# jim-berend/semanticlens

Measured on AMD Instinct MI355X. Metric: images/sec concept-db build, higher is better.
Workload: dtype f32 (encoder GEMMs split-bf16x3, fp32 accumulate)

## Files before the change

include/semanticlens_amd.h:

```cpp
#ifndef SEMANTICLENS_AMD_H
#define SEMANTICLENS_AMD_H

#include <stddef.h>
#include <stdint.h>

#ifdef __cplusplus
extern "C" {
#endif

#define SL_ABI_VERSION 1

#define SL_E_INVALID (-1)
#define SL_E_HIP (-2)
#define SL_E_UNSUPPORTED (-3)

#define SL_F32 0
#define SL_F16 1
#define SL_BF16 2

#define SL_CONV_MAX 0
#define SL_CONV_MEAN 1
#define SL_CONV_SUM 2

#define SL_TOK_MEAN 0
// ... 170 lines not shown
int sl_preprocess_plan_rois(const int32_t* h_hw, const int64_t* h_pixel_offsets, int64_t N, const int64_t* h_index,
                            const int32_t* h_box, int64_t P, int S, int resize_mode, int interp, int64_t* h_plan,
                            int64_t* h_info);

#define SL_RENDER_CROP 0
#define SL_RENDER_OPAQUE 1
#define SL_RENDER_LIGHTEN 2
size_t sl_render_ws_bytes(int64_t B, int64_t H, int64_t W);
int sl_render_heatmaps(const float* d_rel, int64_t B, int64_t Cin, int64_t H, int64_t W, const float* d_img, int kernel_size,
                       float vis_th, float crop_th, double alpha, int style, int rf, float* d_heat, int32_t* d_box,
                       int32_t* d_flags, uint8_t* d_rgb, void* d_ws, size_t ws_bytes, void* stream);
int sl_condition_init(const float* d_act, int64_t B, int64_t C, int64_t S, int64_t sb, int64_t sc, int64_t ss,
                      const int64_t* d_channels, int rf, float* d_out, int64_t ob, int64_t oc, int64_t os, void* stream);

int sl_activation_heat_boxes(const float* d_act, int64_t B, int64_t C, int64_t S, int64_t sb, int64_t sc, int64_t ss,
                             int64_t prefix, int64_t gh, int64_t gw, const int64_t* d_rows, const int64_t* d_channels,
                             int64_t P, int64_t H, int64_t W, int kernel_size, float crop_th, float* d_heat, int32_t* d_box,
                             void* d_ws, size_t ws_bytes, void* stream);
int sl_heat_boxes(const float* d_heat, int64_t P, int64_t H, int64_t W, int kernel_size, float crop_th, int32_t* d_box,
                  void* d_ws, size_t ws_bytes, void* stream);

int sl_batchnorm_infer(const float* d_x, int64_t B, int64_t C, int64_t HW, const float* d_mean, const float* d_var,
                       const float* d_scale, const float* d_bias, double eps, int relu, float* d_y, void* stream);
int sl_batchnorm_infer_add_relu(const float* d_x, const float* d_residual, int64_t B, int64_t C, int64_t HW,
                                const float* d_mean, const float* d_var, const float* d_scale, const float* d_bias,
                                double eps, float* d_y, void* stream);
int sl_batchnorm_infer_add_bn_relu(const float* d_xa, const float* d_mean_a, const float* d_var_a, const float* d_scale_a,
                                   const float* d_bias_a, double eps_a, const float* d_xb, const float* d_mean_b,
                                   const float* d_var_b, const float* d_scale_b, const float* d_bias_b, double eps_b, int64_t B,
                                   int64_t C, int64_t HW, float* d_y, void* stream);
int sl_batchnorm_infer_relu_maxpool(const float* d_x, int64_t B, int64_t C, int64_t H, int64_t W, const float* d_mean,
                                    const float* d_var, const float* d_scale, const float* d_bias, double eps, int kh, int kw,
                                    int sh, int sw, int ph, int pw, float* d_y, void* stream);

int sl_topk_init(float* d_vals, int64_t* d_ids, int64_t R, int64_t k, void* stream);
int sl_topk_merge(float* d_vals, int64_t* d_ids, int64_t R, int64_t k, const float* d_cand, int64_t ld, int64_t B,
                  int64_t id_base, void* d_ws, size_t ws_bytes, void* stream);
size_t sl_topk_merge_ws_bytes(int64_t R, int64_t k, int64_t B);
int sl_topk_merge_states(float* d_vals, int64_t* d_ids, int64_t R, int64_t k, const float* d_other_vals,
                         const int64_t* d_other_ids, int64_t M, void* stream);

int sl_mutualmax_merge(uint64_t* d_row_state, uint64_t* d_col_state, int64_t R, int64_t B, const float* d_cand, int64_t ld,
                       int64_t row_id_base, int64_t col_id_base, void* stream);
int sl_mutualmax_finish(const uint64_t* d_state, int64_t n, float* d_vals, int64_t* d_ids, void* stream);

int sl_segmax_merge(uint64_t* d_state, int64_t state_ld, int64_t G, int64_t R, int64_t B, const float* d_cand, int64_t ld,
                    const int32_t* d_row_seg, int64_t row_id_base, void* stream);

int sl_unionfind_init(int32_t* d_parent, int32_t* d_degree, int32_t* d_status, int64_t n, void* stream);
int sl_threshold_union_merge(int32_t* d_parent, int32_t* d_degree, int32_t* d_status, int64_t n, const float* d_cand, int64_t ld,
                             int64_t R, int64_t B, int64_t row_id_base, int64_t col_id_base, float threshold, void* stream);
int sl_unionfind_flatten(int32_t* d_parent, int64_t n, int32_t* d_status, void* stream);
int sl_group_min_merge(uint32_t* d_state, const int32_t* d_labels, int64_t n, const float* d_cand, int64_t ld, int64_t R, int64_t B,
                       int64_t row_id_base, int64_t col_id_base, void* stream);
int sl_group_min_finish(const uint32_t* d_state, const int32_t* d_labels, int64_t n, float* d_cohesion, void* stream);

int sl_cosine_nt(const float* d_x, int64_t M, const float* d_y, int64_t N, int64_t K, float* d_out, void* d_ws,
                 size_t ws_bytes, void* stream);
size_t sl_cosine_nt_ws_bytes(int64_t M, int64_t N, int64_t K);

#define SL_PROF_REDUCE 0
#define SL_PROF_MERGE 1
#define SL_PROF_GEMM 2
#define SL_PROF_GATHER 3
#define SL_PROF_SCORES 4
#define SL_PROF_BATCHNORM 5
// ... 11 lines not shown
```

semanticlens_amd/_native.py:

```python
from __future__ import annotations

import ctypes
import math
import operator
import os
from pathlib import Path

import torch

_PKG = Path(__file__).resolve().parent
LIB_PATH = _PKG / "lib" / "libsemanticlens_hip.so"

SL_F32, SL_F16, SL_BF16 = 0, 1, 2
SL_CONV_MAX, SL_CONV_MEAN, SL_CONV_SUM = 0, 1, 2
SL_TOK_MEAN, SL_TOK_ABSMEAN, SL_TOK_MAX, SL_TOK_ABSMAX, SL_TOK_TOKEN = 0, 1, 2, 3, 4
SL_TIES_TOTAL, SL_TIES_ATEN = 0, 1
SL_MAX_SLOTS = 16
SL_PROF_REDUCE, SL_PROF_MERGE, SL_PROF_GEMM, SL_PROF_GATHER, SL_PROF_SCORES, SL_PROF_BATCHNORM, SL_PROF_TOPK = 0, 1, 2, 3, 4, 5, 6
SL_ACT_NONE, SL_ACT_GELU, SL_ACT_QUICKGELU, SL_ACT_GELU_TANH = 0, 1, 2, 3
TIE_MODES = {"total": SL_TIES_TOTAL, "aten": SL_TIES_ATEN}
SL_PP_PLAN_STRIDE = 16
PP_RESIZE_MODES = {"shortest": 0, "squash": 1}
PP_INTERP = {"bicubic": 0, "bilinear": 1}
SL_RENDER_CROP, SL_RENDER_OPAQUE, SL_RENDER_LIGHTEN = 0, 1, 2
# ... 60 lines not shown
    "sl_polykmeans_labels": (_int, [_vp, _i64, _i64, _i64, _int, _vp, _int, _vp, _int, _vp, _vp, _vp, _vp, _sz, _vp]),
    "sl_facet_stats": (_int, [_vp, _i64, _i64, _i64, _vp, _int, _vp, _vp, _vp, _vp]),
    "sl_silhouette_ws_bytes": (_sz, [_i64, _i64, _i64]),
    "sl_silhouette": (_int, [_vp, _i64, _i64, _i64, _vp, _int, _int, _int, _vp, _vp, _vp, _sz, _vp]),
    "sl_linear": (_int, [_vp, _i64, _i64, _vp, _i64, _vp, _int, _vp, _vp, _i64, _i64, _i64, _i64, _vp, _vp]),
    "sl_layernorm": (_int, [_vp, _i64, _i64, _i64, _vp, _vp, ctypes.c_float, _vp, _vp, _i64, _vp]),
    "sl_attention": (_int, [_vp, _i64, _i64, _i64, _i64, _int, _vp, _vp, _vp]),
    "sl_attention_bf16x3": (_int, [_vp, _i64, _i64, _i64, _i64, _int, _vp, _vp, _vp]),
    "sl_patchify": (_int, [_vp, _i64, _i64, _i64, _i64, _i64, _vp, _vp, _vp]),
    "sl_attention_pool": (_int, [_vp, _vp, _i64, _i64, _i64, _i64, _i64, _i64, _vp, _vp]),
    "sl_attention_pool_q": (_int, [_vp, _i64, _vp, _i64, _i64, _i64, _i64, _i64, _i64, _vp, _vp]),
    "sl_tokens_from_map": (_int, [_vp, _i64, _i64, _i64, _vp, _vp, _vp]),
    "sl_split_elems": (_sz, [_i64, _i64]),
    "sl_split_bf16": (_int, [_vp, _vp, _i64, _i64, _vp, _vp]),
    "sl_linear_bf16x3": (_int, [_vp, _i64, _i64, _vp, _i64, _vp, _int, _vp, _vp, _vp, _i64, _i64, _i64, _i64, _vp, _vp]),
    "sl_broadcast_row": (_int, [_vp, _vp, _i64, _i64, _i64, _vp, _vp]),
    "sl_embed_tokens": (_int, [_vp, _i64, _vp, _i64, _i64, _i64, _vp, _vp, _vp]),
    "sl_preprocess_plan": (_int, [_vp, _vp, _i64, _int, _int, _int, _vp, _vp]),
    "sl_preprocess": (_int, [_vp, _vp, _i64, _int, _int, _i64, _i64, _vp, _vp, _vp, _vp, _vp, _sz, _vp]),
    "sl_render_ws_bytes": (_sz, [_i64, _i64, _i64]),
    "sl_render_heatmaps": (_int, [_vp, _i64, _i64, _i64, _i64, _vp, _int, ctypes.c_float, ctypes.c_float, ctypes.c_double, _int, _int,
                                  _vp, _vp, _vp, _vp, _vp, _sz, _vp]),
    "sl_condition_init": (_int, [_vp, _i64, _i64, _i64, _i64, _i64, _i64, _vp, _int, _vp, _i64, _i64, _i64, _vp]),
    "sl_preprocess_plan_rois": (_int, [_vp, _vp, _i64, _vp, _vp, _i64, _int, _int, _int, _vp, _vp]),
    "sl_activation_heat_boxes": (_int, [_vp, _i64, _i64, _i64, _i64, _i64, _i64, _i64, _i64, _i64, _vp, _vp, _i64, _i64, _i64, _int,
                                        ctypes.c_float, _vp, _vp, _vp, _sz, _vp]),
    "sl_heat_boxes": (_int, [_vp, _i64, _i64, _i64, _int, ctypes.c_float, _vp, _vp, _sz, _vp]),
    "sl_batchnorm_infer": (_int, [_vp, _i64, _i64, _i64, _vp, _vp, _vp, _vp, ctypes.c_double, _int, _vp, _vp]),
    "sl_batchnorm_infer_add_relu": (_int, [_vp, _vp, _i64, _i64, _i64, _vp, _vp, _vp, _vp, ctypes.c_double, _vp, _vp]),
    "sl_batchnorm_infer_add_bn_relu": (_int, [_vp, _vp, _vp, _vp, _vp, ctypes.c_double, _vp, _vp, _vp, _vp, _vp, ctypes.c_double, _i64, _i64,
                                              _i64, _vp, _vp]),
    "sl_batchnorm_infer_relu_maxpool": (_int, [_vp, _i64, _i64, _i64, _i64, _vp, _vp, _vp, _vp, ctypes.c_double, _int, _int, _int,
                                               _int, _int, _int, _vp, _vp]),
    "sl_topk_init": (_int, [_vp, _vp, _i64, _i64, _vp]),
    "sl_topk_merge": (_int, [_vp, _vp, _i64, _i64, _vp, _i64, _i64, _i64, _vp, _sz, _vp]),
    "sl_topk_merge_ws_bytes": (_sz, [_i64, _i64, _i64]),
    "sl_topk_merge_states": (_int, [_vp, _vp, _i64, _i64, _vp, _vp, _i64, _vp]),
    "sl_mutualmax_merge": (_int, [_vp, _vp, _i64, _i64, _vp, _i64, _i64, _i64, _vp]),
    "sl_mutualmax_finish": (_int, [_vp, _i64, _vp, _vp, _vp]),
    "sl_segmax_merge": (_int, [_vp, _i64, _i64, _i64, _i64, _vp, _i64, _vp, _i64, _vp]),
    "sl_unionfind_init": (_int, [_vp, _vp, _vp, _i64, _vp]),
    "sl_threshold_union_merge": (_int, [_vp, _vp, _vp, _i64, _vp, _i64, _i64, _i64, _i64, _i64, ctypes.c_float, _vp]),
    "sl_unionfind_flatten": (_int, [_vp, _i64, _vp, _vp]),
    "sl_group_min_merge": (_int, [_vp, _vp, _i64, _vp, _i64, _i64, _i64, _i64, _i64, _vp]),
    "sl_group_min_finish": (_int, [_vp, _vp, _i64, _vp, _vp]),
    "sl_cosine_nt": (_int, [_vp, _i64, _vp, _i64, _i64, _vp, _vp, _sz, _vp]),
    "sl_cosine_nt_ws_bytes": (_sz, [_i64, _i64, _i64]),
    "sl_prof_enable": (_int, [_int]),
    "sl_prof_reset": (_int, []),
    "sl_prof_read": (_int, [_int, ctypes.POINTER(ctypes.c_double), ctypes.POINTER(_i64), ctypes.POINTER(ctypes.c_double)]),
}

_lib = None


class NativeLibraryError(RuntimeError):
    """The HIP library is missing or a native call failed."""


def lib():
    global _lib
    if _lib is None:
        path = Path(os.environ.get("SEMANTICLENS_AMD_LIB", LIB_PATH))
        if not path.exists():
            raise NativeLibraryError(
                f"{path} not found. semanticlens_amd has no CPU fallback: build the HIP library first "
# ... 950 lines not shown
        if residual is None:
            rc = lib().sl_batchnorm_infer(_ptr(x), B, C, H * W, _ptr(mean), _ptr(var), _ptr(weight), _ptr(bias), float(eps),
                                          1 if relu else 0, _ptr(out), _stream(x))
        else:
            rc = lib().sl_batchnorm_infer_add_relu(_ptr(x), _ptr(residual), B, C, H * W, _ptr(mean), _ptr(var), _ptr(weight),
                                                   _ptr(bias), float(eps), _ptr(out), _stream(x))
    _check(rc, "sl_batchnorm_infer")
    return out


BN_DUAL_MAX_CHANNELS = 2048


def batchnorm_infer_add_bn_relu(xa: torch.Tensor, bn_a, xb: torch.Tensor, bn_b) -> torch.Tensor:
    if xa.shape != xb.shape or xa.dim() != 4 or xa.device != xb.device:
        raise ValueError(f"batchnorm_infer_add_bn_relu: two 4-D tensors of one shape and device expected, got {tuple(xa.shape)} and "
                         f"{tuple(xb.shape)}")
    B, C, H, W = xa.shape
    for t in (xa, xb):
        if t.dtype is not torch.float32 or not t.is_contiguous() or t.data_ptr() % 16:
            raise ValueError("batchnorm_infer_add_bn_relu: inputs must be contiguous NCHW fp32, 16-byte aligned")
    for p in (*bn_a[:4], *bn_b[:4]):
        if p.dtype is not torch.float32 or p.device != xa.device or not p.is_contiguous() or p.numel() != C:
            raise ValueError(f"batchnorm_infer_add_bn_relu: per-channel tensors must be contiguous fp32 of {C} elements on {xa.device}")
    out = torch.empty_like(xa)
    with _on(xa.device):
        rc = lib().sl_batchnorm_infer_add_bn_relu(_ptr(xa), *(_ptr(p) for p in bn_a[:4]), float(bn_a[4]), _ptr(xb),
                                                  *(_ptr(p) for p in bn_b[:4]), float(bn_b[4]), B, C, H * W, _ptr(out), _stream(xa))
    _check(rc, "sl_batchnorm_infer_add_bn_relu")
    return out


BN_POOL_MAX_WIDTH = 4096
BN_POOL_STAGE_BYTES = 64 * 1024


def bn_pool_supported(kernel_size, stride, padding) -> bool:
    return all(k in (2, 3) and s in (1, 2) and 0 <= p <= k // 2 for k, s, p in zip(kernel_size, stride, padding))


def batchnorm_infer_relu_maxpool(x: torch.Tensor, mean: torch.Tensor, var: torch.Tensor, weight: torch.Tensor, bias: torch.Tensor,
                                 eps: float, kernel_size, stride, padding) -> torch.Tensor:
    B, C, H, W = x.shape
    (kh, kw), (sh, sw), (ph, pw) = kernel_size, stride, padding
    oh, ow = ((n + 2 * p - k) // s + 1 if s > 0 else 0 for n, k, s, p in ((H, kh, sh, ph), (W, kw, sw, pw)))
    out = torch.empty((B, C, max(oh, 0), max(ow, 0)), dtype=x.dtype, device=x.device)
    with _on(x.device):
        rc = lib().sl_batchnorm_infer_relu_maxpool(_ptr(x), B, C, H, W, _ptr(mean), _ptr(var), _ptr(weight), _ptr(bias),
                                                   float(eps), kh, kw, sh, sw, ph, pw, _ptr(out), _stream(x))
    _check(rc, "sl_batchnorm_infer_relu_maxpool")
    return out


def prof_enable(on: bool = True):
    _check(lib().sl_prof_enable(1 if on else 0), "sl_prof_enable")


def prof_reset():
    _check(lib().sl_prof_reset(), "sl_prof_reset")


def prof_read(family: int):
    ms, n, w = ctypes.c_double(), _i64(), ctypes.c_double()
    _check(lib().sl_prof_read(family, ctypes.byref(ms), ctypes.byref(n), ctypes.byref(w)), "sl_prof_read")
    return ms.value, n.value, w.value


POLY2_MAX_N = 128


POLYK_MAX_N = 1024
# ... 522 lines not shown
```

semanticlens_amd/component_visualization/_bn_fuse.py:

```python
from __future__ import annotations

import inspect
import operator
import os
import warnings
import weakref

import torch
import torch.nn as nn
import torch.nn.functional as F

from .. import _native as N

_BN_FORWARD = nn.modules.batchnorm._BatchNorm.forward
_PLANS: "weakref.WeakKeyDictionary[nn.Module, _Plan]" = weakref.WeakKeyDictionary()
_ADDS = (operator.add, operator.iadd, torch.add)
_RELUS = (F.relu, torch.relu, torch.relu_)
_POOL_ARGS = ("kernel_size", "stride", "padding", "dilation", "ceil_mode", "return_indices")


def enabled() -> bool:
    return os.environ.get("SEMANTICLENS_AMD_FUSE_BN", "1") != "0"


# ... 63 lines not shown
            if p is None or p.dtype is not torch.float32 or p.device != x.device or not p.is_contiguous() or p.numel() != x.shape[1]:
                return False
        return True

    def run(self, x, relu: bool, other=None, bn_first: bool = True):
        bn = self.bn
        out = N.batchnorm_infer(x, bn.running_mean, bn.running_var, bn.weight, bn.bias, bn.eps, relu=relu, residual=other)
        key = (relu, other is not None, (x.shape[2] * x.shape[3]) % 4 == 0)
        if key in self.verified:
            return out
        ref = F.batch_norm(x, bn.running_mean, bn.running_var, bn.weight, bn.bias, False, 0.0, bn.eps)
        if other is not None:
            ref = ref + other if bn_first else other + ref
        if relu:
            ref = torch.relu_(ref)
        if torch.equal(out.view(torch.int32), ref.view(torch.int32)):
            self.verified.add(key)
            return out
        self.dropped = True
        warnings.warn(
            f"the fused BatchNorm kernel did not reproduce PyTorch's result bit for bit on a {tuple(x.shape)} input "
            f"(relu={relu}, residual={other is not None}); this BatchNorm2d runs unfused from now on.", RuntimeWarning, stacklevel=3)
        return ref

    def pool_eligible(self, x, params) -> bool:
        (kh, kw), _, (ph, pw) = params
        return (not self.no_pool and x.shape[3] <= N.BN_POOL_MAX_WIDTH and x.shape[2] + 2 * ph >= kh
                and x.shape[3] + 2 * pw >= kw)

    def run_pool(self, x, params):
        bn = self.bn
        k, s, p = params
        out = N.batchnorm_infer_relu_maxpool(x, bn.running_mean, bn.running_var, bn.weight, bn.bias, bn.eps, k, s, p)
        banded = x.shape[2] > N.BN_POOL_STAGE_BYTES // (4 * x.shape[3])
        key = ("pool", params, x.shape[3] % 4 == 0 and out.shape[3] % 4 == 0, banded)
        if key in self.verified:
            return out
        ref = F.batch_norm(x, bn.running_mean, bn.running_var, bn.weight, bn.bias, False, 0.0, bn.eps)
        ref = F.max_pool2d(torch.relu_(ref), k, s, p)
        if out.shape == ref.shape and torch.equal(out.view(torch.int32), ref.view(torch.int32)):
            self.verified.add(key)
            return out
        self.no_pool = True
        warnings.warn(
            f"the fused BatchNorm + ReLU + max-pool kernel did not reproduce PyTorch's result bit for bit on a {tuple(x.shape)} "
            f"input (kernel_size={k}, stride={s}, padding={p}); this max-pool runs unfused from now on.", RuntimeWarning,
            stacklevel=3)
        return ref


def _bn_args(bn: nn.BatchNorm2d):
    return bn.running_mean, bn.running_var, bn.weight, bn.bias, bn.eps


def _bn_forward(site: _Site):
    def forward(x):
        if site.eligible(x):
            return site.run(x, relu=False)
        return _BN_FORWARD(site.bn, x)

    return forward


class _Fused(nn.Module):

    def __init__(self, site: _Site, relu, add=None, bn_first: bool = True):
        super().__init__()
        self.__dict__.update(site=site, relu=relu, add=add, bn_first=bn_first)
# ... 249 lines not shown
```

semanticlens_amd/csrc/batchnorm.hip:

```cpp
#include "common.hpp"

namespace sl {
namespace {

typedef float f4 __attribute__((ext_vector_type(4)));

enum { EPI_PLAIN = 0, EPI_RELU = 1, EPI_ADD_RELU = 2, EPI_ADD_BN_RELU = 3 };
enum { POL_PLAIN = 0, POL_NT_STORE = 1, POL_NT_BOTH = 2 };

constexpr int kBlock = 256;
constexpr int kUnroll = 4;
constexpr int64_t kMaxC = 4096;
constexpr int64_t kMaxCDual = 2048;
constexpr int64_t kLdsPerCu = 160 * 1024;
constexpr size_t kDualResidentFrom = 32 * 1024;
constexpr int64_t kMaxTotal = (int64_t)1 << 31;

__device__ inline float bn_inv_std(float var, double eps) { return __builtin_amdgcn_rsqf(fabsf(var + (float)eps)); }

__device__ inline float bn_value(float x, const f4 k) {
  const float xhat = (x - k.x) * k.y;
  return __fmaf_rn(k.z, xhat, k.w);
}

__device__ inline float relu_clamp(float v) { return v != v ? v : fmaxf(v, 0.f); }

__device__ inline float add_as_aten(float a, float b) {
  float r;
  asm("v_add_f32_e32 %0, %1, %2" : "=v"(r) : "v"(b), "v"(a));
  return r;
}

struct BnParams {
// ... 147 lines not shown
  ProfScope prof(SL_PROF_BATCHNORM, st, (double)total * 4 * passes);
  const int pol = bn_policy(total * 4);
  const size_t lds = (size_t)C * sizeof(f4) * (dual ? 2 : 1);
  const int64_t per_block = (int64_t)kBlock * kUnroll * 4;
  int64_t blocks = (total + per_block - 1) / per_block;
  int64_t per_cu = 8;
  if (dual && lds > kDualResidentFrom) per_cu = kLdsPerCu / (int64_t)lds;
  const int64_t cap = (int64_t)num_cus() * per_cu;
  if (blocks > cap) blocks = cap;
  const dim3 grid((unsigned)blocks);
#define SL_BN_EPI(E_)                                                                                                \
  if (HW % 4 == 0)                                                                                                   \
    launch_policy<E_, true>(prof, pol, grid, lds, st, x, res, y, a, b, (uint32_t)C, (uint32_t)HW, (uint32_t)total);  \
  else                                                                                                               \
    launch_policy<E_, false>(prof, pol, grid, lds, st, x, res, y, a, b, (uint32_t)C, (uint32_t)HW, (uint32_t)total)
  switch (epi) {
    case EPI_PLAIN: SL_BN_EPI(EPI_PLAIN); break;
    case EPI_RELU: SL_BN_EPI(EPI_RELU); break;
    case EPI_ADD_RELU: SL_BN_EPI(EPI_ADD_RELU); break;
    default: SL_BN_EPI(EPI_ADD_BN_RELU); break;
  }
#undef SL_BN_EPI
  SL_CHECK_HIP(hipGetLastError());
  if (dual) {
    ProfScope second(SL_PROF_BATCHNORM, st, 0.0);
    if (second.start) {
      SL_CHECK_HIP(hipEventRecord(second.start, st));
      SL_CHECK_HIP(hipEventRecord(second.stop, st));
    }
  }
  return 0;
}

constexpr int64_t kPoolLds = 64 * 1024;
constexpr int64_t kPoolMaxW = 4096;

struct PoolGeom {
  uint32_t C, H, W, OH, OW, kh, kw, sh, sw, ph, pw;
  uint32_t rows, bands;
  uint32_t nwork;
};

struct PoolBand {
  uint32_t plane, o0, o1, r0, r1;
  f4 k;
};

__device__ inline PoolBand pool_band(const PoolGeom& g, uint32_t work, const float* mean, const float* var, const float* scale,
                                     const float* bias, double eps) {
  PoolBand b;
  b.plane = work / g.bands;
  const uint32_t band = work - b.plane * g.bands, c = b.plane % g.C;
  b.k = f4{mean[c], bn_inv_std(var[c], eps), scale[c], bias[c]};
  b.o0 = band * g.rows;
  b.o1 = b.o0 + g.rows < g.OH ? b.o0 + g.rows : g.OH;
  const int top = (int)(b.o0 * g.sh) - (int)g.ph;
  b.r0 = top > 0 ? (uint32_t)top : 0u;
  const uint32_t bottom = (b.o1 - 1) * g.sh + g.kh - g.ph;
  b.r1 = bottom < g.H ? bottom : g.H;
  return b;
}

__device__ inline float pool_take(float m, float v) { return v > m || v != v ? v : m; }

template <int KW, int SW, int PW, int POL>
__global__ __launch_bounds__(kBlock) void bn_relu_maxpool_kernel(const float* __restrict__ x, float* __restrict__ y,
                                                                 const float* __restrict__ mean, const float* __restrict__ var,
                                                                 const float* __restrict__ scale, const float* __restrict__ bias,
                                                                 double eps, const PoolGeom g) {
  extern __shared__ f4 staged[];
  for (uint32_t work = blockIdx.x; work < g.nwork; work += gridDim.x) {
    const PoolBand b = pool_band(g, work, mean, var, scale, bias, eps);
    const uint32_t w4 = g.W / 4, n4 = (b.r1 - b.r0) * w4;
    const f4* src = reinterpret_cast<const f4*>(x + (size_t)b.plane * g.H * g.W) + (size_t)b.r0 * w4;
    for (uint32_t base = 0; base < n4; base += kBlock * kUnroll) {
      f4 v[kUnroll];
#pragma unroll
      for (int u = 0; u < kUnroll; ++u) {
        const uint32_t i = base + u * kBlock + threadIdx.x;
        if (i < n4) v[u] = ld4<POL>(src + i);
      }
#pragma unroll
      for (int u = 0; u < kUnroll; ++u) {
        const uint32_t i = base + u * kBlock + threadIdx.x;
        if (i < n4) {
          f4 o;
#pragma unroll
          for (int j = 0; j < 4; ++j) o[j] = relu_clamp(bn_value(v[u][j], b.k));
          staged[i] = o;
        }
      }
    }
    __syncthreads();

    constexpr int OFF = PW ? 3 : 0, SPAN = 3 * SW + KW, PIECES = (OFF + SPAN + 3) / 4;
    constexpr float NEG_INF = -__builtin_huge_valf();
    const uint32_t ow4 = g.OW / 4, npieces = (b.o1 - b.o0) * ow4;
    f4* dst = reinterpret_cast<f4*>(y + (size_t)b.plane * g.OH * g.OW);
    for (uint32_t p = threadIdx.x; p < npieces; p += kBlock) {
      const uint32_t orow = p / ow4, q = p - orow * ow4, oh = b.o0 + orow;
      const int col0 = (int)(q * 4 * SW) - (PW ? 4 : 0);
      f4 m = {NEG_INF, NEG_INF, NEG_INF, NEG_INF};
#pragma unroll
      for (int i = 0; i < 3; ++i) {
        const int ih = (int)(oh * g.sh) - (int)g.ph + i;
        if (i < (int)g.kh && ih >= 0 && ih < (int)g.H) {
          const f4* row = staged + (size_t)((uint32_t)ih - b.r0) * w4;
          float t[PIECES * 4];
#pragma unroll
          for (int s = 0; s < PIECES; ++s) {
            const int col = col0 + 4 * s;
            const f4 piece = col >= 0 && col < (int)g.W ? row[col >> 2] : f4{NEG_INF, NEG_INF, NEG_INF, NEG_INF};
#pragma unroll
            for (int j = 0; j < 4; ++j) t[4 * s + j] = piece[j];
          }
#pragma unroll
          for (int o = 0; o < 4; ++o) {
#pragma unroll
            for (int j = 0; j < KW; ++j) m[o] = pool_take(m[o], t[OFF + o * SW + j]);
          }
        }
      }
      st4<POL>(dst + (size_t)oh * ow4 + q, m);
    }
    __syncthreads();
  }
}

template <int POL>
__global__ __launch_bounds__(kBlock) void bn_relu_maxpool_scalar_kernel(const float* __restrict__ x, float* __restrict__ y,
                                                                        const float* __restrict__ mean,
                                                                        const float* __restrict__ var,
                                                                        const float* __restrict__ scale,
                                                                        const float* __restrict__ bias, double eps,
                                                                        const PoolGeom g) {
  extern __shared__ f4 staged[];
  float* rows = reinterpret_cast<float*>(staged);
  for (uint32_t work = blockIdx.x; work < g.nwork; work += gridDim.x) {
    const PoolBand b = pool_band(g, work, mean, var, scale, bias, eps);
    const uint32_t n = (b.r1 - b.r0) * g.W;
    const float* src = x + (size_t)b.plane * g.H * g.W + (size_t)b.r0 * g.W;
#pragma unroll 4
    for (uint32_t i = threadIdx.x; i < n; i += kBlock) rows[i] = relu_clamp(bn_value(ld1<POL>(src + i), b.k));
    __syncthreads();

    const uint32_t nout = (b.o1 - b.o0) * g.OW;
    float* dst = y + (size_t)b.plane * g.OH * g.OW;
    for (uint32_t p = threadIdx.x; p < nout; p += kBlock) {
      const uint32_t orow = p / g.OW, ow = p - orow * g.OW, oh = b.o0 + orow;
      float m = -__builtin_huge_valf();
      for (uint32_t i = 0; i < g.kh; ++i) {
        const int ih = (int)(oh * g.sh) - (int)g.ph + (int)i;
        if (ih < 0 || ih >= (int)g.H) continue;
        for (uint32_t j = 0; j < g.kw; ++j) {
          const int iw = (int)(ow * g.sw) - (int)g.pw + (int)j;
          if (iw < 0 || iw >= (int)g.W) continue;
          m = pool_take(m, rows[((uint32_t)ih - b.r0) * g.W + (uint32_t)iw]);
        }
      }
      st1<POL>(dst + (size_t)oh * g.OW + ow, m);
    }
    __syncthreads();
  }
}

template <int KW, int SW, int PW>
void launch_pool_policy(ProfScope& prof, int pol, dim3 grid, size_t lds, hipStream_t st, const float* x, float* y,
                        const float* mean, const float* var, const float* scale, const float* bias, double eps,
                        const PoolGeom& g) {
#define SL_POOL_LAUNCH(P_) \
  SL_LAUNCH(prof, (bn_relu_maxpool_kernel<KW, SW, PW, P_>), grid, dim3(kBlock), lds, st, x, y, mean, var, scale, bias, eps, g)
  switch (pol) {
    case POL_PLAIN: SL_POOL_LAUNCH(POL_PLAIN); break;
    case POL_NT_STORE: SL_POOL_LAUNCH(POL_NT_STORE); break;
    default: SL_POOL_LAUNCH(POL_NT_BOTH); break;
  }
#undef SL_POOL_LAUNCH
}

int launch_bn_relu_maxpool(const float* x, float* y, const float* mean, const float* var, const float* scale, const float* bias,
                           double eps, int64_t B, int64_t C, int64_t H, int64_t W, int kh, int kw, int sh, int sw, int ph,
                           int pw, hipStream_t st, const char* who) {
  SL_REQUIRE(B >= 0 && C >= 0 && H >= 0 && W >= 0, "%s: negative shape", who);
  SL_REQUIRE((kh == 2 || kh == 3) && (kw == 2 || kw == 3), "%s: kernel size %d x %d is not supported (2 or 3 per axis)", who, kh,
             kw);
  SL_REQUIRE((sh == 1 || sh == 2) && (sw == 1 || sw == 2), "%s: stride %d x %d is not supported (1 or 2 per axis)", who, sh, sw);
  SL_REQUIRE(ph >= 0 && pw >= 0 && ph <= kh / 2 && pw <= kw / 2,
             "%s: padding %d x %d is not supported (at most half the kernel size)", who, ph, pw);
  const int64_t total = B * C * H * W;
  if (total == 0) return 0;
  SL_REQUIRE(H + 2 * ph >= kh && W + 2 * pw >= kw, "%s: a %lld x %lld input is smaller than the pooling window", who,
             (long long)H, (long long)W);
  SL_REQUIRE(x && y && mean && var && scale && bias, "%s: null pointer", who);
  SL_REQUIRE(C <= kMaxC, "%s: %lld channels exceed the supported maximum of %lld", who, (long long)C, (long long)kMaxC);
  SL_REQUIRE(total < kMaxTotal, "%s: %lld elements exceed the supported maximum of 2^31 - 1", who, (long long)total);
  SL_REQUIRE((((uintptr_t)x | (uintptr_t)y) & 15) == 0, "%s: tensors must be 16-byte aligned", who);
  SL_REQUIRE(W <= kPoolMaxW, "%s: rows of %lld elements exceed the supported maximum of %lld", who, (long long)W,
             (long long)kPoolMaxW);
  PoolGeom g;
  g.C = (uint32_t)C, g.H = (uint32_t)H, g.W = (uint32_t)W;
  g.kh = kh, g.kw = kw, g.sh = sh, g.sw = sw, g.ph = ph, g.pw = pw;
  g.OH = (uint32_t)((H + 2 * ph - kh) / sh + 1), g.OW = (uint32_t)((W + 2 * pw - kw) / sw + 1);
  const int64_t fit = kPoolLds / (W * 4);
  int64_t in_rows = H;
  g.rows = g.OH, g.bands = 1;
  if (H > fit) {
    g.rows = (uint32_t)((fit - kh) / sh + 1);
    g.bands = (g.OH + g.rows - 1) / g.rows;
    in_rows = (int64_t)(g.rows - 1) * sh + kh;
  }
  const size_t lds = (size_t)(in_rows * W * 4 + 15) / 16 * 16;
  g.nwork = (uint32_t)(B * C * g.bands);
  int64_t per_cu = kLdsPerCu / (int64_t)lds;
  per_cu = per_cu < 1 ? 1 : per_cu > 8 ? 8 : per_cu;
  const int64_t cap = (int64_t)num_cus() * per_cu;
  const dim3 grid((unsigned)(g.nwork < cap ? g.nwork : cap));
  ProfScope prof(SL_PROF_BATCHNORM, st, ((double)total + (double)B * C * g.OH * g.OW) * 4);
  const int pol = bn_policy(total * 4);
  if (W % 4 == 0 && g.OW % 4 == 0) {
#define SL_POOL_CASE(KW_, SW_, PW_)                                                                              \
  case (KW_ - 2) * 4 + (SW_ - 1) * 2 + PW_:                                                                      \
    launch_pool_policy<KW_, SW_, PW_>(prof, pol, grid, lds, st, x, y, mean, var, scale, bias, eps, g);           \
    break
    switch ((kw - 2) * 4 + (sw - 1) * 2 + pw) {
      SL_POOL_CASE(2, 1, 0);
      SL_POOL_CASE(2, 1, 1);
      SL_POOL_CASE(2, 2, 0);
      SL_POOL_CASE(2, 2, 1);
      SL_POOL_CASE(3, 1, 0);
      SL_POOL_CASE(3, 1, 1);
      SL_POOL_CASE(3, 2, 0);
      default: SL_POOL_CASE(3, 2, 1);
    }
#undef SL_POOL_CASE
  } else {
#define SL_POOL_SCALAR(P_) \
  SL_LAUNCH(prof, (bn_relu_maxpool_scalar_kernel<P_>), grid, dim3(kBlock), lds, st, x, y, mean, var, scale, bias, eps, g)
    switch (pol) {
      case POL_PLAIN: SL_POOL_SCALAR(POL_PLAIN); break;
      case POL_NT_STORE: SL_POOL_SCALAR(POL_NT_STORE); break;
      default: SL_POOL_SCALAR(POL_NT_BOTH); break;
    }
#undef SL_POOL_SCALAR
  }
  SL_CHECK_HIP(hipGetLastError());
  return 0;
}

}
}

using namespace sl;

SL_API int sl_batchnorm_infer(const float* d_x, int64_t B, int64_t C, int64_t HW, const float* d_mean, const float* d_var,
                              const float* d_scale, const float* d_bias, double eps, int relu, float* d_y, void* stream) {
  return launch_batchnorm(relu ? EPI_RELU : EPI_PLAIN, d_x, nullptr, d_y, BnParams{d_mean, d_var, d_scale, d_bias, eps}, BnParams{},
                          B, C, HW, (hipStream_t)stream, "sl_batchnorm_infer");
}

SL_API int sl_batchnorm_infer_add_relu(const float* d_x, const float* d_residual, int64_t B, int64_t C, int64_t HW,
                                       const float* d_mean, const float* d_var, const float* d_scale, const float* d_bias,
                                       double eps, float* d_y, void* stream) {
  return launch_batchnorm(EPI_ADD_RELU, d_x, d_residual, d_y, BnParams{d_mean, d_var, d_scale, d_bias, eps}, BnParams{}, B, C, HW,
                          (hipStream_t)stream, "sl_batchnorm_infer_add_relu");
}

SL_API int sl_batchnorm_infer_add_bn_relu(const float* d_xa, const float* d_mean_a, const float* d_var_a, const float* d_scale_a,
                                          const float* d_bias_a, double eps_a, const float* d_xb, const float* d_mean_b,
                                          const float* d_var_b, const float* d_scale_b, const float* d_bias_b, double eps_b,
                                          int64_t B, int64_t C, int64_t HW, float* d_y, void* stream) {
  return launch_batchnorm(EPI_ADD_BN_RELU, d_xa, d_xb, d_y, BnParams{d_mean_a, d_var_a, d_scale_a, d_bias_a, eps_a},
                          BnParams{d_mean_b, d_var_b, d_scale_b, d_bias_b, eps_b}, B, C, HW, (hipStream_t)stream,
                          "sl_batchnorm_infer_add_bn_relu");
}

SL_API int sl_batchnorm_infer_relu_maxpool(const float* d_x, int64_t B, int64_t C, int64_t H, int64_t W, const float* d_mean,
                                           const float* d_var, const float* d_scale, const float* d_bias, double eps, int kh,
                                           int kw, int sh, int sw, int ph, int pw, float* d_y, void* stream) {
  return launch_bn_relu_maxpool(d_x, d_y, d_mean, d_var, d_scale, d_bias, eps, B, C, H, W, kh, kw, sh, sw, ph, pw,
                                (hipStream_t)stream, "sl_batchnorm_infer_relu_maxpool");
}
```

semanticlens_amd/csrc/common.hpp:

```cpp
#pragma once
#include <hip/hip_ext.h>
#include <hip/hip_runtime.h>

#include <cstdarg>
#include <cstdint>
#include <cstdio>

#include "../../include/semanticlens_amd.h"

#define SL_API extern "C" __attribute__((visibility("default")))

namespace sl {

constexpr int kWave = 64;

void set_error(const char* fmt, ...);
int hip_fail(hipError_t e, const char* what);

#define SL_CHECK_HIP(expr)                                   \
  do {                                                       \
    hipError_t _e = (expr);                                  \
    if (_e != hipSuccess) return ::sl::hip_fail(_e, #expr);  \
  } while (0)

#define SL_REQUIRE(cond, ...)        \
  do {                               \
    if (!(cond)) {                   \
      ::sl::set_error(__VA_ARGS__);  \
      return SL_E_INVALID;           \
    }                                \
  } while (0)

struct ProfScope {
  ProfScope(int family, hipStream_t s, double work);
  hipEvent_t start, stop;
};

#define SL_LAUNCH(prof, kernel, grid, block, shmem, stream, ...)                                             \
  do {                                                                                                       \
    if ((prof).start)                                                                                        \
      hipExtLaunchKernelGGL(kernel, grid, block, shmem, stream, (prof).start, (prof).stop, 0, __VA_ARGS__);  \
    else                                                                                                     \
      hipLaunchKernelGGL(kernel, grid, block, shmem, stream, __VA_ARGS__);                                   \
  } while (0)

enum { OPT_G3_TILE = 0, OPT_F32_TILE, OPT_G3_STRIP_OFF, OPT_COLREDUCE_NW, OPT_BN_POLICY, OPT_G3_SHARED, OPT_COUNT };
int64_t option(int id);

inline int num_cus() {
  static int n = [] {
    int dev = 0, v = 256;
    if (hipGetDevice(&dev) == hipSuccess) (void)hipDeviceGetAttribute(&v, hipDeviceAttributeMultiprocessorCount, dev);
    return v > 0 ? v : 256;
  }();
  return n;
}

inline unsigned stride_grid_256(int64_t n) {
  const int64_t blocks = (n + 255) / 256, cap = (int64_t)num_cus() * 8;
  return (unsigned)(blocks < cap ? blocks : cap);
}

__host__ __device__ inline uint32_t f32_bits(float f) {
  union {
    float f;
    uint32_t u;
  } c;
  c.f = f;
  return c.u;
}
__host__ __device__ inline float bits_f32(uint32_t u) {
  union {
    float f;
    uint32_t u;
  } c;
  c.u = u;
  return c.f;
}

// ... 19 lines not shown
```

semanticlens_amd/csrc/runtime.hip:

```cpp
#include <atomic>
#include <cstdlib>
#include <cstring>
#include <mutex>
#include <string>
#include <vector>

#include "common.hpp"

namespace sl {

static thread_local char g_err[512] = "";

void set_error(const char* fmt, ...) {
  va_list ap;
  va_start(ap, fmt);
  vsnprintf(g_err, sizeof(g_err), fmt, ap);
  va_end(ap);
}

int hip_fail(hipError_t e, const char* what) {
  set_error("HIP error %d (%s) in %s", (int)e, hipGetErrorString(e), what);
  return SL_E_HIP;
}

static const char* const kOptNames[OPT_COUNT] = {"g3_tile", "f32_tile", "g3_strip_off", "colreduce_nw", "bn_policy", "g3_shared"};
static std::atomic<int64_t> g_opts[OPT_COUNT];
static std::once_flag g_opts_once;

static int opt_id(const char* name) {
  for (int i = 0; i < OPT_COUNT; ++i)
    if (name && strcmp(name, kOptNames[i]) == 0) return i;
  return -1;
}

static void opts_from_env() {
  const char* e = getenv("SL_OPTIONS");
  if (!e) return;
  std::string all(e);
  size_t pos = 0;
  while (pos < all.size()) {
    size_t end = all.find(',', pos);
    if (end == std::string::npos) end = all.size();
    const std::string item = all.substr(pos, end - pos);
    const size_t eq = item.find('=');
    if (eq != std::string::npos) {
      const int id = opt_id(item.substr(0, eq).c_str());
      if (id >= 0) g_opts[id].store(atoll(item.c_str() + eq + 1));
    }
    pos = end + 1;
  }
}

int64_t option(int id) {
  std::call_once(g_opts_once, opts_from_env);
  return g_opts[id].load(std::memory_order_relaxed);
}

struct ProfRec {
// ... 4 lines not shown

static std::mutex g_prof_mu;
static bool g_prof_on = false;
static std::vector<ProfRec> g_recs;
static std::vector<ProfRec> g_free_recs;

ProfScope::ProfScope(int family, hipStream_t s, double work) : start(nullptr), stop(nullptr) {
  (void)s;
  if (!g_prof_on) return;
  std::lock_guard<std::mutex> lk(g_prof_mu);
  ProfRec r;
  if (!g_free_recs.empty()) {
    r = g_free_recs.back();
    g_free_recs.pop_back();
  } else {
    if (hipEventCreate(&r.start) != hipSuccess || hipEventCreate(&r.stop) != hipSuccess) return;
  }
  r.fam = family;
  r.work = work;
  g_recs.push_back(r);
  start = r.start;
  stop = r.stop;
}

}

using namespace sl;

SL_API const char* sl_last_error(void) { return g_err; }
SL_API int sl_abi_version(void) { return SL_ABI_VERSION; }

SL_API int sl_set_option(const char* name, int64_t value) {
  const int id = opt_id(name);
  SL_REQUIRE(id >= 0, "sl_set_option: unknown option '%s' (g3_tile, f32_tile, g3_strip_off, colreduce_nw, bn_policy, g3_shared)", name ? name : "(null)");
  (void)option(id);
  g_opts[id].store(value);
  return 0;
}

SL_API int64_t sl_get_option(const char* name) {
  const int id = opt_id(name);
  return id < 0 ? -1 : option(id);
}

SL_API int sl_device_count(void) {
  int n = 0;
  hipError_t e = hipGetDeviceCount(&n);
  if (e != hipSuccess) return hip_fail(e, "hipGetDeviceCount");
  return n;
}

SL_API int sl_prof_enable(int on) {
  std::lock_guard<std::mutex> lk(g_prof_mu);
  g_prof_on = on != 0;
  return 0;
}

SL_API int sl_prof_reset(void) {
  std::lock_guard<std::mutex> lk(g_prof_mu);
  for (auto& r : g_recs) {
    (void)hipEventSynchronize(r.stop);
    g_free_recs.push_back(r);
  }
  g_recs.clear();
  return 0;
}

// ... 20 lines not shown
```

Measured before the change: 7529.

## Prefetch next band in fused BN-ReLU-maxpool and shrink LDS band plan for occupancy

The fused batchnorm+relu+maxpool kernels now issue the global loads for the next band into registers before pooling the current band, which overlaps memory latency with LDS pooling work. The trailing __syncthreads is replaced by an lgkmcnt wait plus a raw barrier. Band planning moves into a shared header: by default each block gets an LDS budget of per-CU LDS divided by 6 instead of the fixed 64KB, with rows balanced across bands, so more blocks can fit per CU. New options allow overriding the LDS budget and the block count. The costs are extra register pressure from the prefetch and more bands, and so more halo rows, for tall planes.

```diff
diff --git a/include/semanticlens_amd.h b/include/semanticlens_amd.h
--- a/include/semanticlens_amd.h
+++ b/include/semanticlens_amd.h
@@ -226,6 +226,7 @@
 int sl_batchnorm_infer_relu_maxpool(const float* d_x, int64_t B, int64_t C, int64_t H, int64_t W, const float* d_mean,
                                     const float* d_var, const float* d_scale, const float* d_bias, double eps, int kh, int kw,
                                     int sh, int sw, int ph, int pw, float* d_y, void* stream);
+int sl_batchnorm_pool_plan(int64_t H, int64_t W, int kh, int sh, int ph, int64_t* rows, int64_t* bands, int64_t* lds_bytes);
 
 int sl_topk_init(float* d_vals, int64_t* d_ids, int64_t R, int64_t k, void* stream);
 int sl_topk_merge(float* d_vals, int64_t* d_ids, int64_t R, int64_t k, const float* d_cand, int64_t ld, int64_t B,
diff --git a/semanticlens_amd/_native.py b/semanticlens_amd/_native.py
--- a/semanticlens_amd/_native.py
+++ b/semanticlens_amd/_native.py
@@ -116,6 +116,7 @@
                                               _i64, _vp, _vp]),
     "sl_batchnorm_infer_relu_maxpool": (_int, [_vp, _i64, _i64, _i64, _i64, _vp, _vp, _vp, _vp, ctypes.c_double, _int, _int, _int,
                                                _int, _int, _int, _vp, _vp]),
+    "sl_batchnorm_pool_plan": (_int, [_i64, _i64, _int, _int, _int, ctypes.POINTER(_i64), ctypes.POINTER(_i64), ctypes.POINTER(_i64)]),
     "sl_topk_init": (_int, [_vp, _vp, _i64, _i64, _vp]),
     "sl_topk_merge": (_int, [_vp, _vp, _i64, _i64, _vp, _i64, _i64, _i64, _vp, _sz, _vp]),
     "sl_topk_merge_ws_bytes": (_sz, [_i64, _i64, _i64]),
@@ -1132,11 +1133,17 @@
 
 
 BN_POOL_MAX_WIDTH = 4096
-BN_POOL_STAGE_BYTES = 64 * 1024
 
 
 def bn_pool_supported(kernel_size, stride, padding) -> bool:
     return all(k in (2, 3) and s in (1, 2) and 0 <= p <= k // 2 for k, s, p in zip(kernel_size, stride, padding))
+
+
+def bn_pool_plan(H: int, W: int, kh: int, sh: int, ph: int) -> tuple[int, int, int]:
+    rows, bands, lds = _i64(), _i64(), _i64()
+    _check(lib().sl_batchnorm_pool_plan(H, W, kh, sh, ph, ctypes.byref(rows), ctypes.byref(bands), ctypes.byref(lds)),
+           "sl_batchnorm_pool_plan")
+    return rows.value, bands.value, lds.value
 
 
 def batchnorm_infer_relu_maxpool(x: torch.Tensor, mean: torch.Tensor, var: torch.Tensor, weight: torch.Tensor, bias: torch.Tensor,
diff --git a/semanticlens_amd/component_visualization/_bn_fuse.py b/semanticlens_amd/component_visualization/_bn_fuse.py
--- a/semanticlens_amd/component_visualization/_bn_fuse.py
+++ b/semanticlens_amd/component_visualization/_bn_fuse.py
@@ -119,8 +119,8 @@
         bn = self.bn
         k, s, p = params
         out = N.batchnorm_infer_relu_maxpool(x, bn.running_mean, bn.running_var, bn.weight, bn.bias, bn.eps, k, s, p)
-        banded = x.shape[2] > N.BN_POOL_STAGE_BYTES // (4 * x.shape[3])
-        key = ("pool", params, x.shape[3] % 4 == 0 and out.shape[3] % 4 == 0, banded)
+        rows, bands, _ = N.bn_pool_plan(x.shape[2], x.shape[3], k[0], s[0], p[0])
+        key = ("pool", params, x.shape[3] % 4 == 0 and out.shape[3] % 4 == 0, bands, rows if bands > 1 else 0)
         if key in self.verified:
             return out
         ref = F.batch_norm(x, bn.running_mean, bn.running_var, bn.weight, bn.bias, False, 0.0, bn.eps)
diff --git a/semanticlens_amd/csrc/batchnorm.hip b/semanticlens_amd/csrc/batchnorm.hip
--- a/semanticlens_amd/csrc/batchnorm.hip
+++ b/semanticlens_amd/csrc/batchnorm.hip
@@ -1,4 +1,6 @@
+#include "bn_pool_plan.hpp"
 #include "common.hpp"
+#include "gemm_ring.hpp"
 
 namespace sl {
 namespace {
@@ -212,8 +214,14 @@
   return 0;
 }
 
-constexpr int64_t kPoolLds = 64 * 1024;
 constexpr int64_t kPoolMaxW = 4096;
+static_assert(kPoolLdsPerCu == kLdsPerCu, "bn_pool_plan.hpp");
+constexpr int64_t kPoolMaxPerCu = 8;
+#ifdef SL_BN_POOL_NO_PREFETCH
+constexpr bool kPoolPrefetch = false;
+#else
+constexpr bool kPoolPrefetch = true;
+#endif
 
 struct PoolGeom {
   uint32_t C, H, W, OH, OW, kh, kw, sh, sw, ph, pw;
@@ -243,35 +251,78 @@
 
 __device__ inline float pool_take(float m, float v) { return v > m || v != v ? v : m; }
 
+__device__ inline const float* pool_src(const float* x, const PoolGeom& g, const PoolBand& b) {
+  return x + (size_t)b.plane * g.H * g.W + (size_t)b.r0 * g.W;
+}
+
+template <int POL>
+__device__ inline void pool_load(f4 (&v)[kUnroll], const float* src, uint32_t base, uint32_t n) {
+#pragma unroll
+  for (int u = 0; u < kUnroll; ++u) {
+    const uint32_t i = base + u * kBlock + threadIdx.x;
+    v[u] = ld4<POL>(reinterpret_cast<const f4*>(src) + (i < n ? i : n - 1));
+  }
+}
+template <int POL>
+__device__ inline void pool_load(float (&v)[kUnroll], const float* src, uint32_t base, uint32_t n) {
+#pragma unroll
+  for (int u = 0; u < kUnroll; ++u) {
+    const uint32_t i = base + u * kBlock + threadIdx.x;
+    v[u] = ld1<POL>(src + (i < n ? i : n - 1));
+  }
+}
+__device__ inline void pool_stage(f4* staged, const f4 (&v)[kUnroll], uint32_t base, uint32_t n, const f4 k) {
+#pragma unroll
+  for (int u = 0; u < kUnroll; ++u) {
+    const uint32_t i = base + u * kBlock + threadIdx.x;
+    if (i < n) {
+      f4 o;
+#pragma unroll
+      for (int j = 0; j < 4; ++j) o[j] = relu_clamp(bn_value(v[u][j], k));
+      staged[i] = o;
+    }
+  }
+}
+__device__ inline void pool_stage(float* rows, const float (&v)[kUnroll], uint32_t base, uint32_t n, const f4 k) {
+#pragma unroll
+  for (int u = 0; u < kUnroll; ++u) {
+    const uint32_t i = base + u * kBlock + threadIdx.x;
+    if (i < n) rows[i] = relu_clamp(bn_value(v[u], k));
+  }
+}
+
+__device__ inline void pool_release_barrier() {
+  asm volatile("s_waitcnt lgkmcnt(0)" ::: "memory");
+  ring::raw_barrier();
+}
+
 template <int KW, int SW, int PW, int POL>
 __global__ __launch_bounds__(kBlock) void bn_relu_maxpool_kernel(const float* __restrict__ x, float* __restrict__ y,
                                                                  const float* __restrict__ mean, const float* __restrict__ var,
                                                                  const float* __restrict__ scale, const float* __restrict__ bias,
                                                                  double eps, const PoolGeom g) {
   extern __shared__ f4 staged[];
-  for (uint32_t work = blockIdx.x; work < g.nwork; work += gridDim.x) {
-    const PoolBand b = pool_band(g, work, mean, var, scale, bias, eps);
-    const uint32_t w4 = g.W / 4, n4 = (b.r1 - b.r0) * w4;
-    const f4* src = reinterpret_cast<const f4*>(x + (size_t)b.plane * g.H * g.W) + (size_t)b.r0 * w4;
-    for (uint32_t base = 0; base < n4; base += kBlock * kUnroll) {
-      f4 v[kUnroll];
-#pragma unroll
-      for (int u = 0; u < kUnroll; ++u) {
-        const uint32_t i = base + u * kBlock + threadIdx.x;
-        if (i < n4) v[u] = ld4<POL>(src + i);
-      }
-#pragma unroll
-      for (int u = 0; u < kUnroll; ++u) {
-        const uint32_t i = base + u * kBlock + threadIdx.x;
-        if (i < n4) {
-          f4 o;
-#pragma unroll
-          for (int j = 0; j < 4; ++j) o[j] = relu_clamp(bn_value(v[u][j], b.k));
-          staged[i] = o;
-        }
-      }
+  const uint32_t w4 = g.W / 4;
+  uint32_t work = blockIdx.x;
+  if (work >= g.nwork) return;
+  PoolBand b = pool_band(g, work, mean, var, scale, bias, eps);
+  f4 v[kUnroll];
+  pool_load<POL>(v, pool_src(x, g, b), 0, (b.r1 - b.r0) * w4);
+  for (;;) {
+    const uint32_t n4 = (b.r1 - b.r0) * w4;
+    pool_stage(staged, v, 0, n4, b.k);
+    for (uint32_t base = kBlock * kUnroll; base < n4; base += kBlock * kUnroll) {
+      pool_load<POL>(v, pool_src(x, g, b), base, n4);
+      pool_stage(staged, v, base, n4, b.k);
     }
     __syncthreads();
+    const uint32_t next = work + gridDim.x;
+    const bool more = next < g.nwork;
+    PoolBand nb = b;
+    if (more) {
+      nb = pool_band(g, next, mean, var, scale, bias, eps);
+      if (kPoolPrefetch) pool_load<POL>(v, pool_src(x, g, nb), 0, (nb.r1 - nb.r0) * w4);
+    }
 
     constexpr int OFF = PW ? 3 : 0, SPAN = 3 * SW + KW, PIECES = (OFF + SPAN + 3) / 4;
     constexpr float NEG_INF = -__builtin_huge_valf();
@@ -303,7 +354,10 @@
       }
       st4<POL>(dst + (size_t)oh * ow4 + q, m);
     }
-    __syncthreads();
+    if (!more) break;
+    pool_release_barrier();
+    b = nb, work = next;
+    if (!kPoolPrefetch) pool_load<POL>(v, pool_src(x, g, b), 0, (b.r1 - b.r0) * w4);
   }
 }
 
@@ -316,13 +370,26 @@
                                                                         const PoolGeom g) {
   extern __shared__ f4 staged[];
   float* rows = reinterpret_cast<float*>(staged);
-  for (uint32_t work = blockIdx.x; work < g.nwork; work += gridDim.x) {
-    const PoolBand b = pool_band(g, work, mean, var, scale, bias, eps);
+  uint32_t work = blockIdx.x;
+  if (work >= g.nwork) return;
+  PoolBand b = pool_band(g, work, mean, var, scale, bias, eps);
+  float v[kUnroll];
+  pool_load<POL>(v, pool_src(x, g, b), 0, (b.r1 - b.r0) * g.W);
+  for (;;) {
     const uint32_t n = (b.r1 - b.r0) * g.W;
-    const float* src = x + (size_t)b.plane * g.H * g.W + (size_t)b.r0 * g.W;
-#pragma unroll 4
-    for (uint32_t i = threadIdx.x; i < n; i += kBlock) rows[i] = relu_clamp(bn_value(ld1<POL>(src + i), b.k));
+    pool_stage(rows, v, 0, n, b.k);
+    for (uint32_t base = kBlock * kUnroll; base < n; base += kBlock * kUnroll) {
+      pool_load<POL>(v, pool_src(x, g, b), base, n);
+      pool_stage(rows, v, base, n, b.k);
+    }
     __syncthreads();
+    const uint32_t next = work + gridDim.x;
+    const bool more = next < g.nwork;
+    PoolBand nb = b;
+    if (more) {
+      nb = pool_band(g, next, mean, var, scale, bias, eps);
+      if (kPoolPrefetch) pool_load<POL>(v, pool_src(x, g, nb), 0, (nb.r1 - nb.r0) * g.W);
+    }
 
     const uint32_t nout = (b.o1 - b.o0) * g.OW;
     float* dst = y + (size_t)b.plane * g.OH * g.OW;
@@ -340,7 +407,10 @@
       }
       st1<POL>(dst + (size_t)oh * g.OW + ow, m);
     }
-    __syncthreads();
+    if (!more) break;
+    pool_release_barrier();
+    b = nb, work = next;
+    if (!kPoolPrefetch) pool_load<POL>(v, pool_src(x, g, b), 0, (b.r1 - b.r0) * g.W);
   }
 }
 
@@ -381,19 +451,15 @@
   g.C = (uint32_t)C, g.H = (uint32_t)H, g.W = (uint32_t)W;
   g.kh = kh, g.kw = kw, g.sh = sh, g.sw = sw, g.ph = ph, g.pw = pw;
   g.OH = (uint32_t)((H + 2 * ph - kh) / sh + 1), g.OW = (uint32_t)((W + 2 * pw - kw) / sw + 1);
-  const int64_t fit = kPoolLds / (W * 4);
-  int64_t in_rows = H;
-  g.rows = g.OH, g.bands = 1;
-  if (H > fit) {
-    g.rows = (uint32_t)((fit - kh) / sh + 1);
-    g.bands = (g.OH + g.rows - 1) / g.rows;
-    in_rows = (int64_t)(g.rows - 1) * sh + kh;
-  }
-  const size_t lds = (size_t)(in_rows * W * 4 + 15) / 16 * 16;
+  const PoolPlan plan = pool_plan(H, W, kh, sh, ph, option(OPT_BN_POOL_LDS));
+  g.rows = plan.rows, g.bands = plan.bands;
+  const size_t lds = plan.lds_bytes;
   g.nwork = (uint32_t)(B * C * g.bands);
   int64_t per_cu = kLdsPerCu / (int64_t)lds;
-  per_cu = per_cu < 1 ? 1 : per_cu > 8 ? 8 : per_cu;
-  const int64_t cap = (int64_t)num_cus() * per_cu;
+  per_cu = per_cu < 1 ? 1 : per_cu > kPoolMaxPerCu ? kPoolMaxPerCu : per_cu;
+  int64_t cap = (int64_t)num_cus() * per_cu;
+  const int64_t forced = option(OPT_BN_POOL_BLOCKS);
+  if (forced > 0 && forced < cap) cap = forced;
   const dim3 grid((unsigned)(g.nwork < cap ? g.nwork : cap));
   ProfScope prof(SL_PROF_BATCHNORM, st, ((double)total + (double)B * C * g.OH * g.OW) * 4);
   const int pol = bn_policy(total * 4);
@@ -460,3 +526,16 @@
   return launch_bn_relu_maxpool(d_x, d_y, d_mean, d_var, d_scale, d_bias, eps, B, C, H, W, kh, kw, sh, sw, ph, pw,
                                 (hipStream_t)stream, "sl_batchnorm_infer_relu_maxpool");
 }
+
+SL_API int sl_batchnorm_pool_plan(int64_t H, int64_t W, int kh, int sh, int ph, int64_t* rows, int64_t* bands,
+                                  int64_t* lds_bytes) {
+  SL_REQUIRE(H >= 1 && W >= 1 && W <= kPoolMaxW, "sl_batchnorm_pool_plan: a %lld x %lld plane is not supported", (long long)H,
+             (long long)W);
+  SL_REQUIRE((kh == 2 || kh == 3) && (sh == 1 || sh == 2) && ph >= 0 && ph <= kh / 2 && H + 2 * ph >= kh,
+             "sl_batchnorm_pool_plan: kernel %d, stride %d, padding %d on %lld rows is not supported", kh, sh, ph, (long long)H);
+  const PoolPlan plan = pool_plan(H, W, kh, sh, ph, option(OPT_BN_POOL_LDS));
+  if (rows) *rows = plan.rows;
+  if (bands) *bands = plan.bands;
+  if (lds_bytes) *lds_bytes = plan.lds_bytes;
+  return 0;
+}
diff --git a/semanticlens_amd/csrc/bn_pool_plan.hpp b/semanticlens_amd/csrc/bn_pool_plan.hpp
--- /dev/null
+++ b/semanticlens_amd/csrc/bn_pool_plan.hpp
@@ -0,0 +1,43 @@
+#pragma once
+#include <cstdint>
+
+#if defined(__HIPCC__)
+#define SL_POOL_PLAN_FN __host__ __device__ inline
+#else
+#define SL_POOL_PLAN_FN inline
+#endif
+
+namespace sl {
+
+constexpr int64_t kPoolLdsMax = 64 * 1024;
+constexpr int64_t kPoolLdsPerCu = 160 * 1024;
+constexpr int64_t kPoolBlocksPerCu = 6;
+
+struct PoolPlan {
+  uint32_t rows, bands;
+  uint32_t in_rows;
+  uint32_t lds_bytes;
+};
+
+SL_POOL_PLAN_FN PoolPlan pool_plan(int64_t H, int64_t W, int kh, int sh, int ph, int64_t budget_bytes) {
+  const int64_t OH = (H + 2 * ph - kh) / sh + 1, row = W * 4, need = kh * row;
+  const bool rule = budget_bytes <= 0;
+  int64_t budget = budget_bytes;
+  if (rule) budget = kPoolLdsPerCu / kPoolBlocksPerCu;
+  if (budget < need) budget = need;
+  if (budget > kPoolLdsMax) budget = kPoolLdsMax;
+  const int64_t fit = budget / row;
+  int64_t rows = OH, bands = 1, in_rows = H;
+  if (H > fit) {
+    rows = (fit - kh) / sh + 1;
+    bands = (OH + rows - 1) / rows;
+    if (rule) rows = (OH + bands - 1) / bands;
+    in_rows = (rows - 1) * sh + kh;
+  }
+  PoolPlan p;
+  p.rows = (uint32_t)rows, p.bands = (uint32_t)bands, p.in_rows = (uint32_t)in_rows;
+  p.lds_bytes = (uint32_t)((in_rows * row + 15) / 16 * 16);
+  return p;
+}
+
+}
diff --git a/semanticlens_amd/csrc/common.hpp b/semanticlens_amd/csrc/common.hpp
--- a/semanticlens_amd/csrc/common.hpp
+++ b/semanticlens_amd/csrc/common.hpp
@@ -44,7 +44,8 @@
       hipLaunchKernelGGL(kernel, grid, block, shmem, stream, __VA_ARGS__);                                   \
   } while (0)
 
-enum { OPT_G3_TILE = 0, OPT_F32_TILE, OPT_G3_STRIP_OFF, OPT_COLREDUCE_NW, OPT_BN_POLICY, OPT_G3_SHARED, OPT_COUNT };
+enum { OPT_G3_TILE = 0, OPT_F32_TILE, OPT_G3_STRIP_OFF, OPT_COLREDUCE_NW, OPT_BN_POLICY, OPT_G3_SHARED, OPT_BN_POOL_LDS,
+       OPT_BN_POOL_BLOCKS, OPT_COUNT };
 int64_t option(int id);
 
 inline int num_cus() {
diff --git a/semanticlens_amd/csrc/runtime.hip b/semanticlens_amd/csrc/runtime.hip
--- a/semanticlens_amd/csrc/runtime.hip
+++ b/semanticlens_amd/csrc/runtime.hip
@@ -23,7 +23,8 @@
   return SL_E_HIP;
 }
 
-static const char* const kOptNames[OPT_COUNT] = {"g3_tile", "f32_tile", "g3_strip_off", "colreduce_nw", "bn_policy", "g3_shared"};
+static const char* const kOptNames[OPT_COUNT] = {"g3_tile", "f32_tile", "g3_strip_off", "colreduce_nw", "bn_policy", "g3_shared",
+                                               "bn_pool_lds", "bn_pool_blocks"};
 static std::atomic<int64_t> g_opts[OPT_COUNT];
 static std::once_flag g_opts_once;
 
@@ -94,7 +95,7 @@
 
 SL_API int sl_set_option(const char* name, int64_t value) {
   const int id = opt_id(name);
-  SL_REQUIRE(id >= 0, "sl_set_option: unknown option '%s' (g3_tile, f32_tile, g3_strip_off, colreduce_nw, bn_policy, g3_shared)", name ? name : "(null)");
+  SL_REQUIRE(id >= 0, "sl_set_option: unknown option '%s' (g3_tile, f32_tile, g3_strip_off, colreduce_nw, bn_policy, g3_shared, bn_pool_lds, bn_pool_blocks)", name ? name : "(null)");
   (void)option(id);
   g_opts[id].store(value);
   return 0;
```

Result: no change. 7543 (median of 5 runs) (+0.2%).
